# I-Mihara/BioDemuX.jl

Hardware: AMD Instinct MI355X
Metric: reads/s demultiplexed (150 bp, 96 barcodes, :semiglobal) at 1/2/4/8 MI355X (higher is better)
Workload: dtype i32

## Files before the change

biodemux.jl_amd/csrc/bdx_wave.hip:

```cpp
#include <atomic>

#include <cstdio>
#include <cstdlib>

#include "bdx_core.h"

#define BDX_BAD_PLAN() (getenv("BDX_TRACE_LAUNCH") ? (void)fprintf(stderr, "[bdx] launch refused at %s:%d\n", __FILE__, __LINE__) : (void)0, hipErrorInvalidValue)

namespace {

struct WaveArgs {
    double max_error_rate, min_delta;
    int counts_stride2;
    const uint8_t *seq;
    const long long *off;
    long long n_reads;
    BdxDevOut out;
    unsigned long long *counts;
    int hist_entries;
    const uint8_t *bitmap;
    int bm_bytes;
    const uint16_t *rank;
    const uint32_t *ent;
    int n_ent;
    const uint32_t *peq8;
    const uint32_t *peq8r;
    int trim0, trim1;
    int need_tb;
    BdxDevStats stats;
    const uint32_t *meta;
    const uint32_t *settle;
    int B;
    int q;
    int span_cap;
    int per_wave;
    int tier;
    double tier_slo;
    double tier_slo1;
    int dual;
    uint32_t *carry_ent;
    uint32_t *list;
    unsigned int *list_count;
    int B0;
    int cw[2];
    uint32_t *cand_out[2];
    uint32_t *wins_out[2];
    uint8_t *wcnt_out[2];
    int short_lb[2];
    int sg;
    int slot;
    int vps, vps_inv;
    int max_len;
    int win_sfe, win_so, win_efe, win_eo;
    int cpr;
    int cpr_inv;
    int hq_cap, sq_cap;
    int ngroups;
    int scan_gpr, scan_gpr_inv;
    int cand_area;
    int ranged;
    BdxDevPass dpass[2];
    const uint32_t *idmap;
    const unsigned int *n_dev;
    uint32_t req;
    int dbg;
};

typedef const __attribute__((address_space(4))) WaveArgs *KArgs;
__device__ __forceinline__ KArgs kargs() {
    uint64_t p = (uint64_t)(uintptr_t)__builtin_amdgcn_kernarg_segment_ptr();
    asm volatile("" : "+s"(p));
    return (KArgs)(uintptr_t)p;
}

enum : uint32_t {
    REQ_BC1 = 1u, REQ_BC2 = 2u, REQ_KS = 4u, REQ_KE = 8u, REQ_PSTART = 16u, REQ_PEND = 32u, REQ_PRAW = 64u, REQ_PBC = 128u,
    REQ_PSCORE = 256u, REQ_PDELTA = 512u, REQ_COUNTS = 1024u,
    REQ_TIER = 2048u, REQ_DELTA = 4096u,
    REQ_PASS = REQ_PSTART | REQ_PEND | REQ_PRAW | REQ_PBC | REQ_PSCORE | REQ_PDELTA
};

#ifdef BDX_TUNING
#define BDX_DBG(bit) (a.dbg & (bit))
#else
#define BDX_DBG(bit) 0
#endif

typedef unsigned int u32x2 __attribute__((ext_vector_type(2)));
typedef unsigned int u32x3 __attribute__((ext_vector_type(3)));

#define WAVE_SYNC()                                          \
    do {                                                     \
        __builtin_amdgcn_fence(__ATOMIC_RELEASE, "wavefront"); \
        __builtin_amdgcn_wave_barrier();                     \
        __builtin_amdgcn_fence(__ATOMIC_ACQUIRE, "wavefront"); \
    } while (0)

template <bool EXACT>
__device__ __forceinline__ void pack16(const u32x4 v, uint32_t &p2, uint32_t &nlo, uint32_t &nhi, uint32_t &sad) {
    constexpr uint32_t CODE_LO = 0x03020100u, CODE_HI = 0x04040404u;
    constexpr uint32_t EXP_LO = 0x47544341u , EXP_HI = 0x4E000000u ;
    uint32_t u[4], t2[4];
#pragma unroll
    for (int w = 0; w < 4; ++w) {
        const uint32_t x = v[w];
        const uint32_t sel = (x >> 1) & 0x07070707u;
        uint32_t n4 = __builtin_amdgcn_perm(CODE_HI, CODE_LO, sel);
        const uint32_t e = __builtin_amdgcn_perm(EXP_HI, EXP_LO, sel);
        if (EXACT) {
            const uint32_t d = x ^ e;
            const uint32_t y = (((d & 0x7F7F7F7Fu) + 0x7F7F7F7Fu) | d) & 0x80808080u;
            const uint32_t m = (y >> 7) * 0xFFu;
            n4 = (n4 & ~m) | (m & 0x04040404u);
        } else {
            sad = __builtin_amdgcn_sad_u8(x, e, sad);
        }
        u[w] = n4 | (n4 >> 4);
        const uint32_t t6 = (x & 0x06060606u) << 5;
        const uint32_t a = t6 | (t6 << 6);
        t2[w] = a | (a << 12);
    }
    nlo = __builtin_amdgcn_perm(u[1], u[0], 0x06040200u);
    nhi = __builtin_amdgcn_perm(u[3], u[2], 0x06040200u);
    const uint32_t lo = __builtin_amdgcn_perm(t2[1], t2[0], 0x0C0C0703u);
    const uint32_t hi = __builtin_amdgcn_perm(t2[3], t2[2], 0x07030C0Cu);
    p2 = lo | hi;
}

template <bool TRACK>
__device__ __forceinline__ uint32_t sweep_step(const uint32_t Eq, uint32_t &Pv, uint32_t &Mv, int &score, int &best) {
    const uint32_t Xv = Eq | Mv;
    const uint32_t ep = Eq & Pv;
    const uint32_t Xh = ((ep + Pv) ^ Pv) | Eq;
    uint32_t Ph = Mv | ~(Xh | Pv);
    uint32_t Mh = Pv & Xh;
    if (TRACK) {
        uint32_t cp, cm;
        Ph = __builtin_addc(Ph, Ph, 0u, &cp);
        Mh = __builtin_addc(Mh, Mh, 0u, &cm);
        score += (int)cp;
        score -= (int)cm;
    } else {
        Ph = Ph + Ph;
        Mh = Mh + Mh;
    }
    Pv = Mh | ~(Xv | Ph);
    Mv = Ph & Xv;
    if (TRACK) best = score < best ? score : best;
    return ep;
}

__device__ __forceinline__ void lds_read8(uint32_t (&d)[8], const uint32_t (&addr)[8]) {
#pragma unroll
    for (int i = 0; i < 8; ++i) asm volatile("ds_read_b32 %0, %1" : "=v"(d[i]) : "v"(addr[i]) : "memory");
}
__device__ __forceinline__ void lds_wait8(uint32_t (&d)[8]) {
    asm volatile("s_waitcnt lgkmcnt(0)"
                 : "+v"(d[0]), "+v"(d[1]), "+v"(d[2]), "+v"(d[3]), "+v"(d[4]), "+v"(d[5]), "+v"(d[6]), "+v"(d[7])
                 :
                 : "memory");
}

template <int TF, int TRACKW>
__device__ __forceinline__ void sweep_block(const uint32_t A0, const uint32_t A1, const uint32_t A2, const uint32_t A3,
                                            const uint32_t pbase, uint32_t &Pv, uint32_t &Mv, int &score, int &best, const int kk1,
                                            uint32_t &inm, uint32_t &inm2, const int ngr) {
    const uint32_t A[4] = {A0, A1, A2, A3};
    uint32_t Eq[2][8];
    const auto issue = [&](const int h) __attribute__((always_inline)) {
        uint32_t addr[8];
#pragma unroll
        for (int jj = 0; jj < 8; ++jj) addr[jj] = pbase + (__builtin_amdgcn_ubfe(A[h], 4 * jj, 3) << 2);
        lds_read8(Eq[h & 1], addr);
    };
    issue(0);
    inm = 0u;
    inm2 = 0u;
#pragma unroll
    for (int h = 0; h < 4; ++h) {
        if (h >= ngr) break;
        lds_wait8(Eq[h & 1]);
        if (h < 3 && h + 1 < ngr) issue(h + 1);
#pragma unroll
        for (int jj = 0; jj < 8; ++jj) {
            const int j = 8 * h + jj;
            if (j < TF) {
                sweep_step<false>(Eq[h & 1][jj], Pv, Mv, score, best);
            } else {
                if (j == TF && TF > 0) score = __builtin_popcount(Pv) - __builtin_popcount(Mv);
                const int best_before = best;
                const uint32_t ep = sweep_step<true>(Eq[h & 1][jj], Pv, Mv, score, best);
                if (TRACKW == 1) inm = __builtin_amdgcn_alignbit(inm, (uint32_t)(score - kk1), 31);
                if (TRACKW >= 2) inm = __builtin_amdgcn_alignbit(inm, (uint32_t)(score - best_before), 31);
                if (TRACKW >= 3) inm2 = __builtin_amdgcn_alignbit(inm2, ep, 31);
            }
        }
    }
    if (TRACKW && ngr < 4) inm <<= 32 - 8 * ngr;
    if (TRACKW >= 3 && ngr < 4) inm2 <<= 32 - 8 * ngr;
}

template <bool REVA>
__device__ __forceinline__ void anchored_block(const uint32_t A0, const uint32_t A1, const uint32_t A2, const uint32_t A3, const uint32_t pbase,
                                               const uint32_t rows, const uint32_t lowbit, uint32_t &Pv, uint32_t &Mv, int &score, const int d,
                                               uint32_t &eqm, uint32_t &inm2, const int ngr) {
    const uint32_t A[4] = {A0, A1, A2, A3};
    uint32_t Eq[2][8];
    const auto issue = [&](const int h) __attribute__((always_inline)) {
        uint32_t addr[8];
#pragma unroll
        for (int jj = 0; jj < 8; ++jj) addr[jj] = pbase + (__builtin_amdgcn_ubfe(A[h], 4 * jj, 3) << 2);
        lds_read8(Eq[h & 1], addr);
    };
    issue(0);
    eqm = 0u;
    inm2 = 0u;
#pragma unroll
    for (int h = 0; h < 4; ++h) {
        if (h >= ngr) break;
        lds_wait8(Eq[h & 1]);
        if (h < 3 && h + 1 < ngr) issue(h + 1);
#pragma unroll
        for (int jj = 0; jj < 8; ++jj) {
            const uint32_t E = REVA ? (Eq[h & 1][jj] & rows) : Eq[h & 1][jj];
            const uint32_t Xv = E | Mv;
            const uint32_t ep = E & Pv;
            const uint32_t Xh = ((ep + Pv) ^ Pv) | E;
            uint32_t Ph = Mv | ~(Xh | Pv);
            uint32_t Mh = Pv & Xh;
            uint32_t cp, cm;
            Ph = __builtin_addc(Ph, Ph, 0u, &cp);
            Mh = __builtin_addc(Mh, Mh, 0u, &cm);
            score += (int)cp;
            score -= (int)cm;
            if (REVA) Ph |= lowbit;
            Pv = Mh | ~(Xv | Ph);
            Mv = Ph & Xv;
            eqm = __builtin_amdgcn_alignbit(eqm, score == d ? 0x80000000u : 0u, 31);
            inm2 = __builtin_amdgcn_alignbit(inm2, ep, 31);
        }
    }
    if (ngr < 4) {
        eqm <<= 32 - 8 * ngr;
        inm2 <<= 32 - 8 * ngr;
    }
}

#ifndef BDX_WAVE_BOUNDS
#define BDX_WAVE_BOUNDS __launch_bounds__(1024)
#endif
template <int RW, int TF, int NV, int Q, bool SPLIT, int KB, int NW, bool MG = false, int KEND = 0, bool GEN = true, bool WINM = false>
__global__ BDX_WAVE_BOUNDS void bdx_wave_kernel(const WaveArgs a) {
    constexpr bool PAIRS = KB > 0;
    constexpr bool KREV = KEND >= 2;
    constexpr bool KALN = KEND == 3;
    constexpr int RCAP = 8;
    const int HQ = a.hq_cap, SQ = PAIRS ? 0 : a.sq_cap;
    constexpr int NREC = PAIRS ? 0 : RW * RCAP;
    extern __shared__ __attribute__((aligned(16))) unsigned char smem_raw[];
    LDS unsigned char *smem = (LDS unsigned char *)smem_raw;
    const int tid = threadIdx.x;
    const int lane = tid & 63;
    const int wv = __builtin_amdgcn_readfirstlane(tid >> 6);
    const int B = a.B;
    constexpr int q = Q;
    const bool ranged = GEN && a.ranged != 0, dual = GEN && a.dual != 0;
    const uint32_t req = a.req;
    static_assert(!WINM || (!PAIRS && !SPLIT && KEND == 0 && GEN), "window mode: the non-split single-seed kernel");
    constexpr bool SCAT = PAIRS || WINM;
    constexpr bool CARRY = PAIRS && !SPLIT && !MG && KB <= 4;
    const uint32_t idmask = (CARRY && a.carry_ent != nullptr) ? 0x3FFFFFFFu : 0xFFFFFFFFu;
    const long long n_reads = (SCAT && a.n_dev) ? (long long)(unsigned int)__builtin_amdgcn_readfirstlane((int)*a.n_dev) : a.n_reads;

    size_t o = 0;
    auto take = [&](size_t bytes) -> LDS unsigned char * {
        LDS unsigned char *p = smem + o;
        o = (o + bytes + 31) & ~(size_t)31;
        return p;
    };
    LDS unsigned char *bm = take((size_t)a.bm_bytes);
    LDS uint16_t *rnk = (LDS uint16_t *)take(PAIRS ? 0 : (size_t)a.bm_bytes / 2);
    LDS uint32_t *ent = (LDS uint32_t *)take((size_t)a.n_ent * 4);
    LDS uint32_t *peq = (LDS uint32_t *)take((size_t)B * 36);
    LDS uint32_t *peqr = (LDS uint32_t *)take(KREV ? (size_t)B * 36 : 0);
    LDS uint32_t *meta = (LDS uint32_t *)take((size_t)B * 4);
    LDS uint32_t *settle = (LDS uint32_t *)take((size_t)B * 4);
    LDS int *hist = (LDS int *)take((size_t)a.hist_entries * 4);
    LDS unsigned char *wbase = smem + o + (size_t)wv * (size_t)a.per_wave;
    constexpr int O_FB = 0;
    constexpr int O_RID = O_FB + ((RW + 1) * 4 + 15) / 16 * 16;
    constexpr int O_RMK = O_RID + NREC * 4;
    constexpr int O_SLOTS = O_RMK + NREC * 4;
    constexpr int O_SCNT = O_SLOTS + RW * 16;
    constexpr int O_FLAG = O_SCNT + RW * 4;
    constexpr int O_WCL1 = O_FLAG + RW * 4;
    constexpr int O_LBUF = O_WCL1 + RW * 4;
    constexpr int O_RL = O_LBUF + 64 * 4;
    constexpr int O_GID = O_RL + (SCAT ? RW * 4 : 0);
    constexpr int O_TN = O_GID + (SCAT ? RW * 4 : 0);
    constexpr int O_SG4 = O_TN + ((WINM || PAIRS) ? RW * 4 : 0);
    constexpr int O_SGID = O_SG4 + (SCAT ? 2 * RW * 16 : 0);
    constexpr int O_STN = O_SGID + (SCAT ? 2 * RW * 4 : 0);
    constexpr int O_IMG2 = O_STN + ((WINM || PAIRS) ? 2 * RW * 4 : 0) + (SCAT ? 16 : 0);
    const int nvec_cap = a.span_cap >> 4;
    LDS int *fb = (LDS int *)(wbase + O_FB);
    LDS uint32_t *rid = (LDS uint32_t *)(wbase + O_RID);
    LDS uint32_t *rmk = (LDS uint32_t *)(wbase + O_RMK);
    LDS uint32_t *slots = (LDS uint32_t *)(wbase + O_SLOTS);
    LDS int *scnt = (LDS int *)(wbase + O_SCNT);
    LDS int *flag = (LDS int *)(wbase + O_FLAG);
    LDS int *wcl1 = (LDS int *)(wbase + O_WCL1);
    LDS uint32_t *lbuf = (LDS uint32_t *)(wbase + O_LBUF);
    LDS int *rl = (LDS int *)(wbase + O_RL);
    LDS uint32_t *gid = (LDS uint32_t *)(wbase + O_GID);
// ... 454 lines not shown
                        for (int tt = 0; tt < P; ++tt) {
                            const uint32_t ea = ad[j - 8 + PL * tt - XLO] + gbase + (uint32_t)(tt * TSTRIDE);
                            if constexpr (NW == 1) {
                                H[tt][0] = *(const LDS uint32_t *)(bm + ea);
                            } else if constexpr (NW == 2) {
                                const u32x2 x = *(const LDS u32x2 *)(bm + ea);
                                H[tt][0] = x[0];
                                H[tt][1] = x[1];
                            } else {
                                const u32x4 x = *(const LDS u32x4 *)(bm + ea);
                                H[tt][0] = x[0];
                                H[tt][1] = x[1];
                                H[tt][2] = x[2];
                                if constexpr (NW == 4) H[tt][3] = x[3];
                            }
                        }
#pragma unroll
                        for (int w = 0; w < NW; ++w) {
                            uint32_t once = H[0][w] | H[1][w];
                            uint32_t twice = H[0][w] & H[1][w];
#pragma unroll
                            for (int tt = 2; tt < P; ++tt) {
                                if (j >= 0) twice |= once & H[tt][w];
                                once |= H[tt][w];
                            }
                            if (j >= 0) {
                                uint32_t F = twice;
                                if constexpr (ND > 0) {
                                    uint32_t near = Ah[0][w];
#pragma unroll
                                    for (int u = 1; u < ND; ++u) near |= Ah[u][w];
                                    F |= once & near;
                                }
                                Fl[w] |= F;
                                dmw[w] = (dmw[w] << 1) | (F != 0u ? 1u : 0u);
                            }
                            if constexpr (ND > 0) Ah[(j + ND) % ND][w] = once;
                        }
                    }
                };
                const auto append = [&](const int grp) __attribute__((always_inline)) {
#pragma unroll
                    for (int w = 0; w < NW; ++w) {
                        uint32_t bits = Fl[w];
                        const int jlo = 15 - (31 - (int)__builtin_clz(dmw[w] | 1u)), jhi = 15 - (int)__builtin_ctz(dmw[w] | 0x10000u);
                        const uint32_t common = ((uint32_t)t << 9) | ((uint32_t)(jhi - jlo) << 13) | ((uint32_t)(16 * c - 8 + jlo + 64) << 17) |
                                                (uint32_t)(128 * grp + 32 * w);
                        unsigned long long mk = __builtin_amdgcn_ballot_w64(bits != 0u);
                        while (mk) {
                            const int k = nhq + (int)__builtin_amdgcn_mbcnt_hi((uint32_t)(mk >> 32), __builtin_amdgcn_mbcnt_lo((uint32_t)mk, 0u));
                            if (bits) {
                                const int bi = __builtin_ctz(bits);
                                bits &= bits - 1u;
                                if (k < HQ) hq[k] = common | (uint32_t)bi;
                            }
                            nhq += (int)__builtin_popcountll(mk);
                            mk = __builtin_amdgcn_ballot_w64(bits != 0u);
                        }
                    }
                };
                if constexpr (KB >= 8) {
                    keys();
                    const uint32_t onm = on ? 0xFFFFFFFFu : 0u;
#pragma unroll
                    for (int j0 = 0; j0 < 16; j0 += 3) {
                        const int j1 = j0 + 2 < 15 ? j0 + 2 : 15;
#pragma unroll
                        for (int w = 0; w < NW; ++w) Fl[w] = dmw[w] = 0u;
#pragma unroll
                        for (int j = j0; j <= j1; ++j) {
#pragma unroll
                            for (int xi = (j == 0 ? 0 : j + PL * (P - 1)); xi <= j + PL * (P - 1); ++xi) ad[xi] = key_addr(xi);
                            uint32_t H[P][NW];
#pragma unroll
                            for (int tt = 0; tt < P; ++tt) {
                                const uint32_t ea = ad[j - 8 + PL * tt - XLO] + (uint32_t)(tt * TSTRIDE);
                                if constexpr (NW <= 2) {
                                    const u32x2 x = *(const LDS u32x2 *)(bm + ea);
                                    H[tt][0] = x[0];
                                    if constexpr (NW == 2) H[tt][1] = x[1];
                                } else {
                                    const u32x4 x = *(const LDS u32x4 *)(bm + ea);
                                    H[tt][0] = x[0];
                                    H[tt][1] = x[1];
                                    H[tt][2] = x[2];
                                    if constexpr (NW == 4) H[tt][3] = x[3];
                                }
                            }
#pragma unroll
                            for (int w = 0; w < NW; ++w) {
                                uint32_t once = H[0][w] | H[1][w];
                                uint32_t twice = H[0][w] & H[1][w];
#pragma unroll
                                for (int tt = 2; tt < P; ++tt) {
                                    twice |= once & H[tt][w];
                                    once |= H[tt][w];
                                }
                                const uint32_t F = twice & onm;
                                Fl[w] |= F;
                                dmw[w] = (dmw[w] << 1) | (F != 0u ? 1u : 0u);
                            }
                        }
#pragma unroll
                        for (int w = 0; w < NW; ++w) {
                            uint32_t bits = Fl[w];
                            const int jlo = j1 - (31 - (int)__builtin_clz(dmw[w] | 1u)), jhi = j1 - (int)__builtin_ctz(dmw[w] | 0x8u);
                            const uint32_t common = ((uint32_t)t << 9) | ((uint32_t)(jhi - jlo) << 13) | ((uint32_t)(16 * c - 8 + jlo + 64) << 17) | (uint32_t)(32 * w);
                            unsigned long long mk = __builtin_amdgcn_ballot_w64(bits != 0u);
                            while (mk) {
                                const int k = nhq + (int)__builtin_amdgcn_mbcnt_hi((uint32_t)(mk >> 32), __builtin_amdgcn_mbcnt_lo((uint32_t)mk, 0u));
                                if (bits) {
                                    const int bi = __builtin_ctz(bits);
                                    bits &= bits - 1u;
                                    if (k < HQ) hq[k] = common | (uint32_t)bi;
                                }
                                nhq += (int)__builtin_popcountll(mk);
                                mk = __builtin_amdgcn_ballot_w64(bits != 0u);
                            }
                        }
                    }
                    if (nhq > HQ - 768) drain();
                } else if constexpr (!MG) {
#pragma unroll
                    for (int w = 0; w < NW; ++w) Fl[w] = dmw[w] = 0u;
                    if (on) {
                        keys();
                        diagonals(0u);
                    }
                    if constexpr (CARRY) {
                        const int st = on ? tn[t] : 0;
                        if (st) {
#pragma unroll
                            for (int w = 0; w < NW; ++w) {
                                const int blo = 32 * w;
                                const uint32_t p0 = a.B0 >= blo + 32 ? 0xFFFFFFFFu : (a.B0 <= blo ? 0u : ((1u << (a.B0 - blo)) - 1u));
                                Fl[w] &= st == 1 ? ~p0 : p0;
                            }
                        }
                    }
                    append(0);
                } else {
                    if (on) keys();
                    for (int grp = 0; grp < a.ngroups; ++grp) {
#pragma unroll
                        for (int w = 0; w < NW; ++w) Fl[w] = dmw[w] = 0u;
                        if (on) diagonals((uint32_t)grp * (uint32_t)(P * TSTRIDE));
                        append(grp);
                        if (nhq > HQ - 384) drain();
                    }
                }
            }
        } else {
            constexpr uint32_t AMASK = ((1u << (2 * Q - 5)) - 1u) << 2;
            constexpr uint32_t KMASK = (1u << (2 * Q)) - 1u;
            uint32_t amask = AMASK, kmask = KMASK, emask = 0x55555555u;
            asm volatile("" : "+v"(amask), "+v"(kmask), "+v"(emask));
            int gpr = (GEN && ranged) ? a.scan_gpr : 0;
            const int npw = (GEN && a.B0 < B) ? 2 : 1;
            if (gpr > 0) {
                bool over = false;
                if (lane < nr) {
#pragma unroll
                    for (int p = 0; p < 2; ++p) {
                        if (p < npw) {
                            const int s0 = fb[lane] + wwin[(2 * p) * RW + lane], s1 = fb[lane] + wwin[(2 * p + 1) * RW + lane] - Q;
                            over = over || (s1 >= s0 && (s1 >> 4) - (s0 >> 4) + 1 > gpr);
                        }
                    }
                }
                if (__builtin_amdgcn_ballot_w64(over)) gpr = 0;
            }
            const int nscan = BDX_DBG(8) ? 0 : (gpr > 0 ? nr * npw * gpr : nvec);
            for (int g0i = 0; g0i < nscan; g0i += 64) {
                int g = g0i + lane;
                bool ong = g < nscan;
                uint32_t keep = emask;
                if (gpr > 0) {
                    const int i = g0i + lane;
                    const int tw = ong ? (int)(((uint32_t)i * (uint32_t)a.scan_gpr_inv) >> 16) : 0;
                    const int t = npw == 2 ? tw >> 1 : tw, which = npw == 2 ? tw & 1 : 0;
                    int s0 = fb[t] + wwin[(2 * which) * RW + t];
                    const int f1 = fb[t + 1];
                    g = (s0 >> 4) + (i - tw * gpr);
                    if (which) {
                        const int c0 = (((fb[t] + wwin[t]) >> 4) + gpr) << 4;
                        const int a0 = fb[t] + wwin[t];
                        if (s0 >= a0 && s0 < c0) s0 = c0;
                    }
                    const int below = s0 - 16 * g, above = f1 - 16 * g;
                    ong = ong && above > 0 && g < nvec;
                    const int b2 = below > 0 ? 2 * (below > 16 ? 16 : below) : 0, a2 = above < 16 ? 2 * (above < 0 ? 0 : above) : 32;
                    keep = (b2 >= 32 ? 0u : 0xFFFFFFFFu << b2) & (a2 >= 32 ? 0xFFFFFFFFu : (1u << a2) - 1u) & 0x55555555u;
                }
                uint32_t hits = 0;
                uint32_t w0 = 0, w1 = 0;
                if (ong) {
                    w0 = img2[g];
                    w1 = img2[g + 1];
                    const uint32_t wm = __builtin_amdgcn_alignbit(w1, w0, 16);
                    uint32_t Wk[16];
#pragma unroll
                    for (int i = 0; i < 16; ++i) Wk[i] = i == 0 ? w0 : (i <= 8 ? w0 >> (2 * i) : wm >> (2 * (i - 8)));
#pragma unroll
                    for (int h = 0; h < 2; ++h) {
                        uint32_t word[8], addr[8];
#pragma unroll
                        for (int i = 0; i < 8; ++i) addr[i] = (Wk[8 * h + i] >> 3) & amask;
                        lds_read8(word, addr);
                        lds_wait8(word);
#pragma unroll
                        for (int i = 0; i < 8; ++i) hits = __builtin_amdgcn_alignbit(word[i] >> (Wk[8 * h + i] & 31u), hits, 2);
                    }
                    hits &= keep;
                }
                unsigned long long mk = __builtin_amdgcn_ballot_w64(hits != 0u);
                if (mk) {
                    const uint32_t nl = (uint32_t)__builtin_popcount(hits);
                    uint32_t k = (uint32_t)nhq;
                    for (uint32_t j = 1; mk; ++j) {
                        k = __builtin_amdgcn_mbcnt_hi((uint32_t)(mk >> 32), __builtin_amdgcn_mbcnt_lo((uint32_t)mk, k));
                        nhq += (int)__builtin_popcountll(mk);
                        mk = __builtin_amdgcn_ballot_w64(nl > j);
                    }
                    if (nhq <= HQ && hits) {
                        const uint32_t gp = (uint32_t)g << 20;
                        LDS uint32_t *dst = hq + k;
                        do {
                            const uint32_t i2 = (uint32_t)__builtin_ctz(hits);
                            hits &= hits - 1u;
                            const uint32_t ph = gp + (i2 << 15), kw = __builtin_amdgcn_alignbit(w1, w0, i2);
                            *dst = Q == 8 ? __builtin_amdgcn_perm(ph, kw, 0x07060100u) : ph | (kw & kmask);
                            __builtin_amdgcn_sched_barrier(0);
                            ++dst;
                        } while (hits);
                    }
                }
            }
        }
        if constexpr (PAIRS) drain();
        WAVE_SYNC();
        const bool hq_ok = PAIRS ? !hq_over : nhq <= HQ;
        const int nh = (hq_ok && !BDX_DBG(4) && !PAIRS) ? nhq : 0;

        int ns = 0;
        if constexpr (!PAIRS) {
            const int fb0 = fb[0];
            const float rinv = ulen > 0 ? 1.0f / (float)ulen : 0.0f;
            const float ginv = total > 0 ? (float)nr / (float)total : 0.0f;
            for (int k0 = 0; k0 < nh; k0 += 64) {
                const int k = k0 + lane;
                int new0 = -1, new1 = -1;
                if (k < nh) {
                    const uint32_t h = hq[k];
                    const int pos = (int)(h >> 16);
                    const uint32_t key = h & 0xFFFFu;
                    int t;
                    bool ok = true;
                    if (SCAT) {
                        t = (int)(((uint32_t)(pos >> 4) * (uint32_t)a.vps_inv) >> 16);
                        ok = t < nr;
                        t = ok ? t : 0;
                    } else if (ulen > 0) {
                        const int x = pos - fb0;
                        t = (int)((float)x * rinv);
                        t = t * ulen > x ? t - 1 : t;
                        t = (t + 1) * ulen <= x ? t + 1 : t;
                        ok = x >= 0 && t < nr;
                        t = ok ? t : 0;
                    } else {
                        t = (int)((float)pos * ginv);
                        t = t > nr - 1 ? nr - 1 : t;
                        while (t > 0 && pos < fb[t]) --t;
                        while (t < nr - 1 && pos >= fb[t + 1]) ++t;
                    }
                    const int f0 = fb[t];
                    const int p = pos - f0, n = SCAT ? rl[t] : fb[t + 1] - f0;
                    if (ok && p >= 0 && p + q <= n) {
                        const uint32_t wi = key >> 5;
                        uint32_t idx = (uint32_t)rnk[wi] + (uint32_t)__builtin_popcount(((const LDS uint32_t *)bm)[wi] & ((1u << (key & 31u)) - 1u));
                        do {
                            const uint32_t e = ent[idx];
                            idx = e >> 16;
                            bool inwin = true;
                            if (ranged) {
                                const bool second_b = (int)(e & 2047u) - 1 >= a.B0;
                                inwin = p >= wwin[(second_b ? 2 : 0) * RW + t] && p + q <= wwin[(second_b ? 3 : 1) * RW + t];
                            }
                            if (inwin) {
                                const uint32_t pb = e & 2047u;
                                const int kk = (int)((meta[pb - 1u] >> 8) & 255u);
                                const int diag = p - (int)((e >> 11) & 31u);
                                const uint32_t mine = pb | ((uint32_t)(diag + 64) << 16);
                                int rs = (int)((pb + (uint32_t)(diag >> 3)) & (RCAP - 1));
                                bool placed = false;
                                for (int tries = 0; tries < RCAP && !placed; ++tries) {
                                    LDS uint32_t *id = rid + t * RCAP + rs;
                                    uint32_t old = *id;
                                    bool opened = false;
                                    if (old == 0u) {
                                        uint32_t expect = 0u;
                                        __hip_atomic_compare_exchange_strong(id, &expect, mine, __ATOMIC_RELAXED, __ATOMIC_RELAXED, __HIP_MEMORY_SCOPE_WORKGROUP);
                                        opened = expect == 0u;
                                        old = opened ? mine : expect;
                                    }
                                    const int dd = diag - ((int)(old >> 16) - 64);
                                    if ((old & 0xFFFFu) == pb && dd >= -kk && dd <= kk) {
                                        __hip_atomic_fetch_or(&rmk[t * RCAP + rs], 1u << (dd + kk), __ATOMIC_RELAXED, __HIP_MEMORY_SCOPE_WORKGROUP);
                                        placed = true;
                                        if (opened) {
                                            if (new0 < 0)
                                                new0 = t * RCAP + rs;
                                            else if (new1 < 0)
                                                new1 = t * RCAP + rs;
                                            else {
                                                if (flag[t] != 1) flag[t] = 2;
                                                rid[t * RCAP + rs] = 0u;
                                                rmk[t * RCAP + rs] = 0u;
                                            }
                                        }
                                    }
                                    rs = (rs + 1) & (RCAP - 1);
                                }
                                if (!placed && flag[t] != 1) flag[t] = 2;
                            }
                        } while (idx != 0u);
                    }
                }
#pragma unroll
                for (int layer = 0; layer < 2; ++layer) {
                    const int nw = layer == 0 ? new0 : new1;
                    const unsigned long long mk = __builtin_amdgcn_ballot_w64(nw >= 0);
                    if (mk) {
                        const int kq = ns + (int)__builtin_amdgcn_mbcnt_hi((uint32_t)(mk >> 32), __builtin_amdgcn_mbcnt_lo((uint32_t)mk, 0u));
                        if (nw >= 0) {
                            if (kq < SQ) {
                                recq[kq] = (uint32_t)nw;
                            } else {
                                if (flag[nw / RCAP] != 1) flag[nw / RCAP] = 2;
                                rid[nw] = 0u;
                                rmk[nw] = 0u;
                            }
                        }
                        ns += (int)__builtin_popcountll(mk);
                    }
                }
            }
        }
        ns = ns < SQ ? ns : SQ;
        WAVE_SYNC();

        if constexpr (!PAIRS)
        for (int s0 = 0; s0 < ns; s0 += 64) {
            const int k = s0 + lane;
            bool valid = k < ns;
            const uint32_t rslot = valid ? recq[k] : 0u;
            const uint32_t id = valid ? rid[rslot] : 0u;
            const uint32_t dmk = valid ? rmk[rslot] : 0u;
            if (valid) {
                rid[rslot] = 0u;
                rmk[rslot] = 0u;
            }
            valid = valid && id != 0u && dmk != 0u;
            const int t = (int)(rslot / RCAP), b = valid ? (int)(id & 0xFFFFu) - 1 : 0;
            int lo = 0, hi = 0;
            if (valid) {
                const uint32_t mt = meta[b];
                const int mm = (int)(mt & 255u), kk = (int)((mt >> 8) & 255u);
                const int d0 = (int)(id >> 16) - 64;
                const int dmin = d0 + __builtin_ctz(dmk) - kk, dmax = d0 + (31 - __builtin_clz(dmk)) - kk;
                const int n = rlen(t);
                lo = dmin - kk - 1;
                hi = dmax + mm + kk + 1;
                int wlo = 0, whi = n;
                if (ranged) {
                    wlo = wwin[(b >= a.B0 ? 2 : 0) * RW + t];
                    whi = wwin[(b >= a.B0 ? 3 : 1) * RW + t];
                }
                lo = lo < wlo ? wlo : lo;
                hi = hi > whi ? whi : hi;
            }
            sweep_lane(valid, t, b, lo, hi);
        }
        WAVE_SYNC();
        if (SPLIT || !PAIRS) {
            unsigned long long fm = !tile_ok ? 0ull
                                    : SPLIT  ? __builtin_amdgcn_ballot_w64(lane < nr && (flag[lane] != 0 || !hq_ok))
                                             : ((hq_ok && !(a.dbg & (1 << 30))) ? __builtin_amdgcn_ballot_w64(lane < nr && flag[lane] == 2) : 0ull);
            while (fm) {
                const int t = (int)__builtin_ctzll(fm);
                fm &= fm - 1ull;
                if (lane == 0) {
                    scnt[t] = 0;
                    wcl1[t] = 0;
                    flag[t] = 0;
                    if (SPLIT)
                        for (int w = 0; w < cwt; ++w) cand[t * cwt + w] = 0u;
                }
                WAVE_SYNC();
                const int n = rlen(t);
                for (int b0 = 0; b0 < B; b0 += 64) {
                    const int b = b0 + lane < B ? b0 + lane : 0;
                    const bool valid = b0 + lane < B && ((meta[b] >> 8) & 255u) != 255u;
                    sweep_lane(valid, t, b, win_lo(t, b >= a.B0), win_hi(t, b >= a.B0, n));
                }
                WAVE_SYNC();
            }
        }

        if (SPLIT) {
            if (lane < nr && !BDX_DBG(1)) {
                const long long rid_g = PAIRS ? (long long)gid[lane] : r0 + lane;
                const bool usable = tile_ok && !flag[lane] && (!PAIRS || rl[lane] >= 0);
#pragma unroll
                for (int pass = 0; pass < 2; ++pass) {
                    if (pass == 1 && a.cw[1] == 0) break;
                    const int cwp = pass ? a.cw[1] : a.cw[0];
                    uint32_t *dst = (pass ? a.cand_out[1] : a.cand_out[0]) + rid_g * cwp;
                    for (int w = 0; w < cwp; ++w) dst[w] = usable ? cand[lane * cwt + (pass ? a.cw[0] : 0) + w] : 0xFFFFFFFFu;
                    const int c = pass ? wcl1[lane] : scnt[lane];
                    (pass ? a.wcnt_out[1] : a.wcnt_out[0])[rid_g] = (unsigned char)((usable && c <= BDX_WCAP) ? c : 255);
                }
            }
            WAVE_SYNC();
            tile = tile_next;
            geo = geo_next;
            ov = ov_next;
            ov_next = ov_after;
            so_next = so_after;
            iv_next = iv_after;
            iv_after = iv_after2;
            par ^= 1;
            continue;
// ... 766 lines not shown
```

Baseline: 8.999 billion.

## Software-pipeline k-mer scan LDS reads and use umulhi for hit-to-read mapping

The k-mer scan loop now prefetches the next trip's image words while the current trip's 16 bitmap lookups are in flight. Both halves of those lookups are issued before a single wait, instead of waiting per half. The hit-to-read mapping replaces the float reciprocal with two correction steps by a fixed-point umulhi division when read length exceeds one. The bitmap and rank loads are hoisted ahead of the read lookup, and the read bounds are fetched with paired LDS reads. The aim is to hide LDS latency and cut ALU work, at the cost of more registers and reads issued for lanes that end up masked.

```diff
diff --git a/biodemux.jl_amd/csrc/bdx_wave.hip b/biodemux.jl_amd/csrc/bdx_wave.hip
--- a/biodemux.jl_amd/csrc/bdx_wave.hip
+++ b/biodemux.jl_amd/csrc/bdx_wave.hip
@@ -160,6 +160,15 @@
                  :
                  : "memory");
 }
+__device__ __forceinline__ void lds_name8(uint32_t (&d)[8]) {
+    asm volatile("" : "+v"(d[0]), "+v"(d[1]), "+v"(d[2]), "+v"(d[3]), "+v"(d[4]), "+v"(d[5]), "+v"(d[6]), "+v"(d[7]) : : "memory");
+}
+__device__ __forceinline__ void lds_name2(uint32_t &d0, uint32_t &d1) { asm volatile("" : "+v"(d0), "+v"(d1) : : "memory"); }
+__device__ __forceinline__ void lds_read2(uint32_t &d0, uint32_t &d1, const uint32_t addr) {
+    asm volatile("ds_read_b32 %0, %1" : "=v"(d0) : "v"(addr) : "memory");
+    asm volatile("ds_read_b32 %0, %1 offset:4" : "=v"(d1) : "v"(addr) : "memory");
+}
+__device__ __forceinline__ void lds_wait2(uint32_t &d0, uint32_t &d1) { asm volatile("s_waitcnt lgkmcnt(0)" : "+v"(d0), "+v"(d1) : : "memory"); }
 
 template <int TF, int TRACKW>
 __device__ __forceinline__ void sweep_block(const uint32_t A0, const uint32_t A1, const uint32_t A2, const uint32_t A3,
@@ -939,10 +948,10 @@
                 if (__builtin_amdgcn_ballot_w64(over)) gpr = 0;
             }
             const int nscan = BDX_DBG(8) ? 0 : (gpr > 0 ? nr * npw * gpr : nvec);
-            for (int g0i = 0; g0i < nscan; g0i += 64) {
-                int g = g0i + lane;
+            const auto trip_head = [&](const int g0i, int &g, uint32_t &keep) __attribute__((always_inline)) -> int {
+                g = g0i + lane;
                 bool ong = g < nscan;
-                uint32_t keep = emask;
+                keep = emask;
                 if (gpr > 0) {
                     const int i = g0i + lane;
                     const int tw = ong ? (int)(((uint32_t)i * (uint32_t)a.scan_gpr_inv) >> 16) : 0;
@@ -956,28 +965,47 @@
                         if (s0 >= a0 && s0 < c0) s0 = c0;
                     }
                     const int below = s0 - 16 * g, above = f1 - 16 * g;
-                    ong = ong && above > 0 && g < nvec;
+                    ong = ong && above > 0 && g >= 0 && g < nvec;
                     const int b2 = below > 0 ? 2 * (below > 16 ? 16 : below) : 0, a2 = above < 16 ? 2 * (above < 0 ? 0 : above) : 32;
                     keep = (b2 >= 32 ? 0u : 0xFFFFFFFFu << b2) & (a2 >= 32 ? 0xFFFFFFFFu : (1u << a2) - 1u) & 0x55555555u;
                 }
+                keep = ong ? keep : 0u;
+                return ong ? g : 0;
+            };
+            const uint32_t img2_base = (uint32_t)(uintptr_t)img2;
+            int g = 0;
+            uint32_t keep = 0u, w0 = 0u, w1 = 0u;
+            if (nscan > 0) {
+                const uint32_t ia = img2_base + 4u * (uint32_t)trip_head(0, g, keep);
+                lds_read2(w0, w1, ia);
+                lds_wait2(w0, w1);
+            }
+            for (int g0i = 0; g0i < nscan; g0i += 64) {
+                int gn = 0;
+                uint32_t keepn = 0u, wn0 = 0u, wn1 = 0u;
+                const uint32_t ian = img2_base + 4u * (uint32_t)trip_head(g0i + 64 < nscan ? g0i + 64 : nscan, gn, keepn);
                 uint32_t hits = 0;
-                uint32_t w0 = 0, w1 = 0;
-                if (ong) {
-                    w0 = img2[g];
-                    w1 = img2[g + 1];
+                {
                     const uint32_t wm = __builtin_amdgcn_alignbit(w1, w0, 16);
                     uint32_t Wk[16];
 #pragma unroll
                     for (int i = 0; i < 16; ++i) Wk[i] = i == 0 ? w0 : (i <= 8 ? w0 >> (2 * i) : wm >> (2 * (i - 8)));
+                    uint32_t word[2][8];
 #pragma unroll
                     for (int h = 0; h < 2; ++h) {
-                        uint32_t word[8], addr[8];
+                        uint32_t addr[8];
 #pragma unroll
                         for (int i = 0; i < 8; ++i) addr[i] = (Wk[8 * h + i] >> 3) & amask;
-                        lds_read8(word, addr);
-                        lds_wait8(word);
-#pragma unroll
-                        for (int i = 0; i < 8; ++i) hits = __builtin_amdgcn_alignbit(word[i] >> (Wk[8 * h + i] & 31u), hits, 2);
+                        lds_read8(word[h], addr);
+                    }
+                    lds_read2(wn0, wn1, ian);
+                    lds_wait8(word[0]);
+                    lds_name8(word[1]);
+                    lds_name2(wn0, wn1);
+#pragma unroll
+                    for (int h = 0; h < 2; ++h) {
+#pragma unroll
+                        for (int i = 0; i < 8; ++i) hits = __builtin_amdgcn_alignbit(word[h][i] >> (Wk[8 * h + i] & 31u), hits, 2);
                     }
                     hits &= keep;
                 }
@@ -1003,6 +1031,10 @@
                         } while (hits);
                     }
                 }
+                g = gn;
+                keep = keepn;
+                w0 = wn0;
+                w1 = wn1;
             }
         }
         if constexpr (PAIRS) drain();
@@ -1013,7 +1045,10 @@
         int ns = 0;
         if constexpr (!PAIRS) {
             const int fb0 = fb[0];
-            const float rinv = ulen > 0 ? 1.0f / (float)ulen : 0.0f;
+            const uint32_t fb_base = (uint32_t)(uintptr_t)fb;
+            static_assert(NV * 1024 <= 65536, "hit -> read by umulhi: a tile's span is below 2^16 bases");
+            const uint32_t uinv = ulen > 1 ? 0xFFFFFFFFu / (uint32_t)ulen + 1u : 0u;
+            const float rinv = ulen == 1 ? 1.0f : 0.0f;
             const float ginv = total > 0 ? (float)nr / (float)total : 0.0f;
             for (int k0 = 0; k0 < nh; k0 += 64) {
                 const int k = k0 + lane;
@@ -1022,6 +1057,8 @@
                     const uint32_t h = hq[k];
                     const int pos = (int)(h >> 16);
                     const uint32_t key = h & 0xFFFFu;
+                    const uint32_t wi = key >> 5;
+                    const uint32_t bmw = ((const LDS uint32_t *)bm)[wi], rk = (uint32_t)rnk[wi];
                     int t;
                     bool ok = true;
                     if (SCAT) {
@@ -1030,9 +1067,13 @@
                         t = ok ? t : 0;
                     } else if (ulen > 0) {
                         const int x = pos - fb0;
-                        t = (int)((float)x * rinv);
-                        t = t * ulen > x ? t - 1 : t;
-                        t = (t + 1) * ulen <= x ? t + 1 : t;
+                        if (ulen > 1) {
+                            t = (int)__umulhi((uint32_t)x, uinv);
+                        } else {
+                            t = (int)((float)x * rinv);
+                            t = t * ulen > x ? t - 1 : t;
+                            t = (t + 1) * ulen <= x ? t + 1 : t;
+                        }
                         ok = x >= 0 && t < nr;
                         t = ok ? t : 0;
                     } else {
@@ -1041,11 +1082,18 @@
                         while (t > 0 && pos < fb[t]) --t;
                         while (t < nr - 1 && pos >= fb[t + 1]) ++t;
                     }
-                    const int f0 = fb[t];
-                    const int p = pos - f0, n = SCAT ? rl[t] : fb[t + 1] - f0;
+                    uint32_t f0u, f1u;
+                    if (SCAT) {
+                        f0u = (uint32_t)fb[t];
+                        f1u = f0u + (uint32_t)rl[t];
+                    } else {
+                        lds_read2(f0u, f1u, fb_base + 4u * (uint32_t)t);
+                        lds_wait2(f0u, f1u);
+                    }
+                    const int f0 = (int)f0u;
+                    const int p = pos - f0, n = (int)f1u - f0;
                     if (ok && p >= 0 && p + q <= n) {
-                        const uint32_t wi = key >> 5;
-                        uint32_t idx = (uint32_t)rnk[wi] + (uint32_t)__builtin_popcount(((const LDS uint32_t *)bm)[wi] & ((1u << (key & 31u)) - 1u));
+                        uint32_t idx = rk + (uint32_t)__builtin_popcount(bmw & ((1u << (key & 31u)) - 1u));
                         do {
                             const uint32_t e = ent[idx];
                             idx = e >> 16;
```

Result: no change. 8.946 billion (-0.6%).

## Batch seed-scan over five vector groups and defer key extraction to verify stage

Applied to the files above, without the earlier changes.

In the non-generic path, the seed scan now handles five 64-lane groups per iteration. Hit bits from pairs of groups are packed into interleaved words, so the ballot/mbcnt queue allocation runs once per batch instead of once per group. Queue entries now hold a compact group/bit index rather than position plus key. The verify stage rebuilds the position and re-reads the k-mer key from img2, which adds extra LDS/global reads there. The aim is to amortize the per-iteration cross-lane append overhead, at the cost of more registers and more complex hit encoding.

```diff
diff --git a/biodemux.jl_amd/csrc/bdx_wave.hip b/biodemux.jl_amd/csrc/bdx_wave.hip
--- a/biodemux.jl_amd/csrc/bdx_wave.hip
+++ b/biodemux.jl_amd/csrc/bdx_wave.hip
@@ -920,9 +920,8 @@
             }
         } else {
             constexpr uint32_t AMASK = ((1u << (2 * Q - 5)) - 1u) << 2;
-            constexpr uint32_t KMASK = (1u << (2 * Q)) - 1u;
-            uint32_t amask = AMASK, kmask = KMASK, emask = 0x55555555u;
-            asm volatile("" : "+v"(amask), "+v"(kmask), "+v"(emask));
+            uint32_t amask = AMASK, emask = 0x55555555u;
+            asm volatile("" : "+v"(amask), "+v"(emask));
             int gpr = (GEN && ranged) ? a.scan_gpr : 0;
             const int npw = (GEN && a.B0 < B) ? 2 : 1;
             if (gpr > 0) {
@@ -939,68 +938,103 @@
                 if (__builtin_amdgcn_ballot_w64(over)) gpr = 0;
             }
             const int nscan = BDX_DBG(8) ? 0 : (gpr > 0 ? nr * npw * gpr : nvec);
-            for (int g0i = 0; g0i < nscan; g0i += 64) {
-                int g = g0i + lane;
-                bool ong = g < nscan;
-                uint32_t keep = emask;
-                if (gpr > 0) {
-                    const int i = g0i + lane;
-                    const int tw = ong ? (int)(((uint32_t)i * (uint32_t)a.scan_gpr_inv) >> 16) : 0;
-                    const int t = npw == 2 ? tw >> 1 : tw, which = npw == 2 ? tw & 1 : 0;
-                    int s0 = fb[t] + wwin[(2 * which) * RW + t];
-                    const int f1 = fb[t + 1];
-                    g = (s0 >> 4) + (i - tw * gpr);
-                    if (which) {
-                        const int c0 = (((fb[t] + wwin[t]) >> 4) + gpr) << 4;
-                        const int a0 = fb[t] + wwin[t];
-                        if (s0 >= a0 && s0 < c0) s0 = c0;
-                    }
-                    const int below = s0 - 16 * g, above = f1 - 16 * g;
-                    ong = ong && above > 0 && g < nvec;
-                    const int b2 = below > 0 ? 2 * (below > 16 ? 16 : below) : 0, a2 = above < 16 ? 2 * (above < 0 ? 0 : above) : 32;
-                    keep = (b2 >= 32 ? 0u : 0xFFFFFFFFu << b2) & (a2 >= 32 ? 0xFFFFFFFFu : (1u << a2) - 1u) & 0x55555555u;
-                }
-                uint32_t hits = 0;
-                uint32_t w0 = 0, w1 = 0;
-                if (ong) {
-                    w0 = img2[g];
-                    w1 = img2[g + 1];
-                    const uint32_t wm = __builtin_amdgcn_alignbit(w1, w0, 16);
-                    uint32_t Wk[16];
-#pragma unroll
-                    for (int i = 0; i < 16; ++i) Wk[i] = i == 0 ? w0 : (i <= 8 ? w0 >> (2 * i) : wm >> (2 * (i - 8)));
-#pragma unroll
-                    for (int h = 0; h < 2; ++h) {
-                        uint32_t word[8], addr[8];
-#pragma unroll
-                        for (int i = 0; i < 8; ++i) addr[i] = (Wk[8 * h + i] >> 3) & amask;
-                        lds_read8(word, addr);
-                        lds_wait8(word);
-#pragma unroll
-                        for (int i = 0; i < 8; ++i) hits = __builtin_amdgcn_alignbit(word[i] >> (Wk[8 * h + i] & 31u), hits, 2);
-                    }
-                    hits &= keep;
-                }
-                unsigned long long mk = __builtin_amdgcn_ballot_w64(hits != 0u);
+            constexpr int KT = GEN ? 1 : 5;
+            constexpr uint32_t KMASK = (1u << (2 * Q)) - 1u;
+            for (int r0i = 0; r0i < nscan; r0i += 64 * KT) {
+                uint32_t hm[KT];
+                uint32_t w0 = 0, w1 = 0, gp = 0;
+#pragma unroll
+                for (int u = 0; u < KT; ++u) {
+                    hm[u] = 0u;
+                    const int g0i = r0i + 64 * u;
+                    if (g0i >= nscan) continue;
+                    int g = g0i + lane;
+                    bool ong = g < nscan;
+                    uint32_t keep = emask;
+                    if (gpr > 0) {
+                        const int i = g0i + lane;
+                        const int tw = ong ? (int)(((uint32_t)i * (uint32_t)a.scan_gpr_inv) >> 16) : 0;
+                        const int t = npw == 2 ? tw >> 1 : tw, which = npw == 2 ? tw & 1 : 0;
+                        int s0 = fb[t] + wwin[(2 * which) * RW + t];
+                        const int f1 = fb[t + 1];
+                        g = (s0 >> 4) + (i - tw * gpr);
+                        if (which) {
+                            const int c0 = (((fb[t] + wwin[t]) >> 4) + gpr) << 4;
+                            const int a0 = fb[t] + wwin[t];
+                            if (s0 >= a0 && s0 < c0) s0 = c0;
+                        }
+                        const int below = s0 - 16 * g, above = f1 - 16 * g;
+                        ong = ong && above > 0 && g < nvec;
+                        const int b2 = below > 0 ? 2 * (below > 16 ? 16 : below) : 0, a2 = above < 16 ? 2 * (above < 0 ? 0 : above) : 32;
+                        keep = (b2 >= 32 ? 0u : 0xFFFFFFFFu << b2) & (a2 >= 32 ? 0xFFFFFFFFu : (1u << a2) - 1u) & 0x55555555u;
+                    }
+                    if (ong) {
+                        uint32_t hits = 0;
+                        w0 = img2[g];
+                        w1 = img2[g + 1];
+                        gp = (uint32_t)g << 20;
+                        const uint32_t wm = __builtin_amdgcn_alignbit(w1, w0, 16);
+                        uint32_t Wk[16];
+#pragma unroll
+                        for (int i2 = 0; i2 < 16; ++i2) Wk[i2] = i2 == 0 ? w0 : (i2 <= 8 ? w0 >> (2 * i2) : wm >> (2 * (i2 - 8)));
+#pragma unroll
+                        for (int h = 0; h < 2; ++h) {
+                            uint32_t word[8], addr[8];
+#pragma unroll
+                            for (int i2 = 0; i2 < 8; ++i2) addr[i2] = (Wk[8 * h + i2] >> 3) & amask;
+                            lds_read8(word, addr);
+                            lds_wait8(word);
+#pragma unroll
+                            for (int i2 = 0; i2 < 8; ++i2) hits = __builtin_amdgcn_alignbit(word[i2] >> (Wk[8 * h + i2] & 31u), hits, 2);
+                        }
+                        hm[u] = hits & keep;
+                    }
+                }
+                constexpr int KW = (KT + 1) / 2;
+                uint32_t cw[KW];
+#pragma unroll
+                for (int j = 0; j < KW; ++j) cw[j] = hm[2 * j] | (2 * j + 1 < KT ? hm[2 * j + 1] << 1 : 0u);
+                uint32_t nl = 0;
+#pragma unroll
+                for (int j = 0; j < KW; ++j) nl += (uint32_t)__builtin_popcount(cw[j]);
+                unsigned long long mk = __builtin_amdgcn_ballot_w64(nl != 0u);
                 if (mk) {
-                    const uint32_t nl = (uint32_t)__builtin_popcount(hits);
                     uint32_t k = (uint32_t)nhq;
                     for (uint32_t j = 1; mk; ++j) {
                         k = __builtin_amdgcn_mbcnt_hi((uint32_t)(mk >> 32), __builtin_amdgcn_mbcnt_lo((uint32_t)mk, k));
                         nhq += (int)__builtin_popcountll(mk);
                         mk = __builtin_amdgcn_ballot_w64(nl > j);
                     }
-                    if (nhq <= HQ && hits) {
-                        const uint32_t gp = (uint32_t)g << 20;
+                    if (nhq <= HQ && nl) {
+                        uint32_t cd[KW];
+#pragma unroll
+                        for (int j = 0; j < KW; ++j) cd[j] = (uint32_t)(r0i + 128 * j + lane) << 5;
+                        static_assert(KW == 1 || KW == 3, "the hand-over is written for three words");
+                        if constexpr (KW == 3) {
+                            if (cw[1] == 0u) {
+                                cw[1] = cw[2];
+                                cd[1] = cd[2];
+                            }
+                        }
                         LDS uint32_t *dst = hq + k;
                         do {
-                            const uint32_t i2 = (uint32_t)__builtin_ctz(hits);
-                            hits &= hits - 1u;
-                            const uint32_t ph = gp + (i2 << 15), kw = __builtin_amdgcn_alignbit(w1, w0, i2);
-                            *dst = Q == 8 ? __builtin_amdgcn_perm(ph, kw, 0x07060100u) : ph | (kw & kmask);
+                            const bool z = cw[0] == 0u;
+#pragma unroll
+                            for (int j = 0; j < KW - 1; ++j) {
+                                cw[j] = z ? cw[j + 1] : cw[j];
+                                cd[j] = z ? cd[j + 1] : cd[j];
+                            }
+                            const uint32_t b = (uint32_t)__builtin_ctz(cw[0]);
+                            cw[0] &= cw[0] - 1u;
+                            if constexpr (KT == 1) {
+                                const uint32_t ph = gp + (b << 15), kw = __builtin_amdgcn_alignbit(w1, w0, b);
+                                *dst = Q == 8 ? __builtin_amdgcn_perm(ph, kw, 0x07060100u) : ph | (kw & KMASK);
+                            } else {
+                                *dst = cd[0] + b;
+                            }
                             __builtin_amdgcn_sched_barrier(0);
                             ++dst;
-                        } while (hits);
+                        } while (KT == 1 ? cw[0] != 0u : --nl != 0u);
                     }
                 }
             }
@@ -1020,8 +1054,14 @@
                 int new0 = -1, new1 = -1;
                 if (k < nh) {
                     const uint32_t h = hq[k];
-                    const int pos = (int)(h >> 16);
-                    const uint32_t key = h & 0xFFFFu;
+                    int pos = (int)(h >> 16);
+                    uint32_t key = h & 0xFFFFu;
+                    if constexpr (!GEN) {
+                        const int hg = (int)(h >> 5) + (int)((h & 1u) << 6);
+                        const uint32_t i2 = h & 30u;
+                        pos = 16 * hg + (int)(i2 >> 1);
+                        key = __builtin_amdgcn_alignbit(img2[hg + 1], img2[hg], i2) & ((1u << (2 * Q)) - 1u);
+                    }
                     int t;
                     bool ok = true;
                     if (SCAT) {
```

Result: faster. 8.931 billion before, 9.239 billion after (median of 6 runs) (+3.5%).
